# SyamVangara/multigrid-petsc

Hardware: AMD Instinct MI355X
Metric: fp64 DOF-updates/sec per V-cycle at 1024^3 (higher is better)
Workload: dtype f64

## Files before the change

### include/mgk.h

```cpp
#ifndef MGK_H
#define MGK_H
#include <stddef.h>
#ifdef __cplusplus
extern "C" {
#endif

#define MGK_XOFF 16
#define MGK_EINVAL  10001
#define MGK_ENOGPU  10002
#define MGK_ECOMM   10003

typedef struct mgk_ctx mgk_ctx;

typedef struct mgk_geom {
    int  dim;
    int  nx, ny, nz;
    int  pitch;
    long plane;
    long org;
    long total;
} mgk_geom;

int  mgk_geom_init(mgk_geom *g, int dim, int nx, int ny, int nz);

// ... 348 lines not shown
    MGK_TUNE_J2_REG_PRED       = 36,
    MGK_TUNE_J2_RING_PRED      = 37,
    MGK_TUNE_PJ2D_WAVES        = 38,
    MGK_TUNE_J2_RING_OLD       = 39,
    MGK_TUNE_SRR_TY2           = 40,
    MGK_TUNE_SRR_TY4           = 41,
    MGK_TUNE_J2_ZERO_RINGB     = 45,
    MGK_TUNE_PJ2_COPY          = 46,
    MGK_TUNE_J3_2D_MARCH       = 50,
    MGK_TUNE_J3_2D_CHUNK4      = 51,
    MGK_TUNE_J3_2D_CHUNK8      = 52,
    MGK_TUNE_DISPATCH_ORDER    = 53,
    MGK_TUNE_XCD_ORDER         = 54,
    MGK_TUNE_RR2D_MARCH        = 55,
    MGK_TUNE_RR2D_SHORT        = 56,
    MGK_TUNE_RESERVED_57       = 57,
    MGK_TUNE_J3_2D_ODD_DOWN    = 58,
    MGK_TUNE_J3_2D_ALL_DOWN    = 59,
    MGK_TUNE_J3_2D_STORE_PLAIN = 60,
    MGK_TUNE_J3_2D_STORE_NT    = 61,
    MGK_TUNE_J3_3D_TY2         = 62,
    MGK_TUNE_J3_3D_TY3         = 63,
    MGK_TUNE_J3_3D_ROWWISE     = 64,
    MGK_TUNE_NO_EXACT_FMA      = 65
};

void mgk_set_tuning(int variant, int zchunk);

#ifdef __cplusplus
}
#endif
#endif
```

### multigrid_petsc_amd/csrc/mg_solver.c

```c
#include "mgsolve.h"
#include "mg_comm.h"
#include "mg_solver_internal.h"
#include <math.h>
#include <stdio.h>
#include <stdlib.h>
#include <string.h>
#include <time.h>

#define MG_PI 3.14159265358979323846
static __thread char g_mgerr[512] = "ok";
const char *mg_last_error(void) { return g_mgerr; }
static int mgfail(int code, const char *what) {
    snprintf(g_mgerr, sizeof(g_mgerr), "%s (code %d; kernel layer: %s)", what, code, mgk_last_error());
    return code;
}

typedef struct mg_ops {
    int esz;
    int (*jacobi_range)(mgk_ctx *, const mgk_geom *, const double *, double, double, const void *, const void *, void *, int, int, void *);
    int (*jacobi_zero)(mgk_ctx *, const mgk_geom *, double, double, const void *, void *, void *);
    int (*residual)(mgk_ctx *, const mgk_geom *, const double *, const void *, const void *, void *, void *);
    int (*restrict_fw)(mgk_ctx *, const mgk_geom *, const mgk_geom *, const void *, void *, void *);
    int (*prolong_add)(mgk_ctx *, const mgk_geom *, const mgk_geom *, const void *, void *, void *);
    int (*prolong_jacobi)(mgk_ctx *, const mgk_geom *, const mgk_geom *, const double *, double, double, const void *, const void *, const void *, void *, void *);
// ... 295 lines not shown
    if (s->cfg.rtol <= 0) s->cfg.rtol = 1.e-7;
    if (s->cfg.dist_min_n <= 0) {
        const int n0 = mg_grid_n(cfg->npts, 0);
        s->cfg.dist_min_n = n0 < 255 ? n0 : 255;
    }
    if (s->cfg.fuse < 0) s->cfg.fuse = MG_FUSE_DEFAULT;
    if (s->cfg.pair_min_n <= 0) s->cfg.pair_min_n = (cfg->dim == 3) ? 255 : 2047;
    if (s->cfg.pc_type == MG_PC_RBGS) s->cfg.fuse &= ~(MG_FUSE_POINT_JACOBI_PASSES & ~MG_FUSE_PROLONG_SWEEP);
    else if (s->cfg.pc_type != MG_PC_JACOBI) s->cfg.fuse &= ~MG_FUSE_POINT_JACOBI_PASSES;
    if (s->cfg.mesh) s->cfg.fuse &= ~MG_FUSE_NO_ROW_TABLE_FORM;
    if (s->cfg.overlap < 0) s->cfg.overlap = 1;
    if (s->cfg.graph < 0) s->cfg.graph = 1;
    if (s->cfg.nranks < 1) s->cfg.nranks = 1;
    s->comm = comm;
    s->levels = cfg->levels;
    int rc = mgk_ctx_create(&s->ctx, cfg->device);
    if (rc) { free(s); return mgfail(rc, "mg_solver_create: mgk_ctx_create"); }
    if (s->cfg.slab_chunk < 0) {
        const char *e = getenv("MG_SLAB_CHUNK");
        const int quarter = (mg_grid_n(cfg->npts, 0) / (s->cfg.nranks > 0 ? s->cfg.nranks : 1)) / 4;
        s->cfg.slab_chunk = (e && *e && atoi(e) >= 0) ? atoi(e) : (quarter > 32 ? quarter : 32);
    }
    if (s->cfg.nranks > 1 && s->cfg.dim == 3) mgk_ctx_set_chunk_planes(s->ctx, s->cfg.slab_chunk);

    s->ldist = 0;
    if (s->cfg.nranks > 1) {
        for (int l = 0; l < s->levels; l++) {
            int n = mg_grid_n(cfg->npts, l);
            if (n >= s->cfg.dist_min_n && n >= 2 * s->cfg.nranks) s->ldist = l + 1; else break;
        }
        if (s->ldist == 0) { mg_solver_destroy(s); return mgfail(MGK_EINVAL, "mg_solver_create: grid too small to distribute"); }
        s->zstart = (int *)calloc(s->cfg.nranks + 1, sizeof(int));
        for (int r = 0; r < s->cfg.nranks; r++) {
            int a, b;
            if (mg_slab_range(cfg->npts, s->ldist, s->ldist, r, s->cfg.nranks, &a, &b)) {
                mg_solver_destroy(s);
                return mgfail(MGK_EINVAL, "mg_solver_create: too many ranks for this grid");
            }
            s->zstart[r] = a; s->zstart[r + 1] = b;
        }
    }

    const int mixed = (cfg->precision == MG_PREC_MIXED);
    for (int l = 0; l < s->levels; l++) {
        mg_level *L = &s->L[l];
        L->n = mg_grid_n(cfg->npts, l);
// ... 576 lines not shown
    }
    CHK(O->restrict_fw(s->ctx, &F->g, &Cq->g, F->rv, Cq->b, NULL));
    return 0;
}

static int prolong_from(mg_solver *s, int P, int l) {
    mg_level *Lf = &s->L[l], *Lc = &s->L[l + 1];
    mg_fset *F = &Lf->f[P], *Cq = &Lc->f[P];
    const mg_ops *O = &OPS[P];
    if (F->u_ghost_pending) CHK(ensure_u_ghosts(s, P, Lf));
    if (Lf->distributed && !Lc->distributed) {
        mgk_geom gc = Cq->g;
        int c0 = s->zstart[s->cfg.rank], c1 = s->zstart[s->cfg.rank + 1];
        gc.nz = c1 - c0;
        CHK(O->prolong_add(s->ctx, &F->g, &gc, (char *)Cq->u + (size_t)O->esz * (size_t)c0 * (size_t)Cq->g.plane, F->u, NULL));
    } else {
        CHK(ensure_u_ghosts(s, P, Lc));
        CHK(O->prolong_add(s->ctx, &F->g, &Cq->g, Cq->u, F->u, NULL));
    }
    F->u_ghost_ok = 0;
    return 0;
}

static int pjp_ok(const mg_solver *s, int P) {
    const mg_level *L = &s->L[0];
    const int need = MG_FUSE_PROLONG_PAIR | MG_FUSE_SWEEP_RESTRICT | MG_FUSE_PAIRS | MG_FUSE_NORM_SWEEP | MG_FUSE_PROLONG_SWEEP | MG_FUSE_RESNORM;
    if ((s->cfg.fuse & need) != need || P != 0 || s->cfg.dim != 3 || s->cfg.mesh || s->cfg.ksp_type != MG_KSP_RICHARDSON) return 0;
    if (s->cfg.v[0] != 3 || s->levels < 2 || s->lgraph == 1 || L->n < s->cfg.pair_min_n || s->last_cycle) return 0;
    if (L->distributed) {
        const mg_level *Lc = &s->L[1];
        const int hi = s->cfg.rank < s->cfg.nranks - 1;
        if (!(s->cfg.fuse & MG_FUSE_PROLONG_PAIR_SLAB) || !Lc->distributed || !L->f[0].far || !Lc->f[0].far || L->nz_min < 8 || Lc->nz_min < 4) return 0;
        return mgk_prolong_jacobi2_slab_ok_f64(&L->f[0].g, &Lc->f[0].g, hi) && mgk_jacobi2_sumsq_ok_f64(&L->f[0].g);
    }
    return mgk_prolong_jacobi2_ok_f64(&L->f[0].g, &s->L[1].f[0].g) && mgk_jacobi2_sumsq_ok_f64(&L->f[0].g);
}
static int finalize_iterate(mg_solver *s) {
    if (!s->iterate_behind) return 0;
    mg_level *L = &s->L[0];
    mg_fset *F = &L->f[0];
    if (L->distributed) {
        CHK(ensure_u_ghosts(s, 0, L));
        CHK(mgk_jacobi_range_f64(s->ctx, &F->g, L->coef, L->dinv, s->cfg.scale, (const double *)F->b, (const double *)F->u, (double *)F->tmp, 0, F->g.nz, NULL));
    } else
    CHK(mgk_jacobi_f64(s->ctx, &F->g, L->coef, L->dinv, s->cfg.scale, (const double *)F->b, (const double *)F->u, (double *)F->tmp, NULL));
    swap_ptr(&F->u, &F->tmp);
    mgi_u_rewritten(F);
    s->iterate_behind = 0; s->spec_valid = 0;
    return 0;
}

// ... 342 lines not shown
        if (s->sweep_owed && L->distributed) {
            const int nz = F->g.nz, lo = s->cfg.rank > 0, hi = s->cfg.rank < s->cfg.nranks - 1;
            void *cs = mgk_stream_compute(s->ctx), *ms = mgk_stream_comm(s->ctx);
            int n1 = 0, n2 = 0, n3 = 0;
            CHK(group_exchange(s, 0, F, 0));
#define J2M(z0, z1, off, np) mgk_jacobi2_sumsq_mid_slab_f64(s->ctx, &F->g, &F->gfar, L->coef, L->dinv, s->cfg.scale, (const double *)F->b, (const double *)F->u, \
                                (double *)F->tmp, (const double *)F->far, lo, hi, z0, z1, off, np, cs)
            const int split = s->cfg.overlap && nz >= 6;
            if (split) {
                void *t = prof_begin_kind(s, 0, 1);
                int rc2 = J2M(2, nz - 2, 0, &n1);
                prof_end(s, t);
                CHK(rc2);
            }
            CHK(mgk_stream_wait(s->ctx, cs, ms));
            F->u_ghost_pending = 0; F->u_ghost_ok = 1; F->b_ghost_ok = 1;
            if (split) { CHK(J2M(0, 2, n1, &n2)); CHK(J2M(nz - 2, nz, n1 + n2, &n3)); }
            else CHK(J2M(0, nz, 0, &n1));
#undef J2M
            CHK(mgk_partials_finish(s->ctx, n1 + n2 + n3, &ss, NULL));
            s->sweep_owed = 0; s->iterate_behind = 1; s->spec_valid = 1;
            goto norm_done;
        }
        if (s->sweep_owed) {
            void *t = prof_begin_kind(s, 0, 1);
            int rc2 = mgk_jacobi2_sumsq_mid_f64(s->ctx, &F->g, L->coef, L->dinv, s->cfg.scale, (const double *)F->b, (const double *)F->u,
                                                (double *)F->tmp, &ss, NULL);
            prof_end(s, t);
            CHK(rc2);
            s->sweep_owed = 0; s->iterate_behind = 1; s->spec_valid = 1;
            goto norm_done;
        }
        if (jnorm && L->distributed && s->cfg.dim == 3 && (s->cfg.fuse & MG_FUSE_SWEEP_RESTRICT) && (s->cfg.fuse & MG_FUSE_PAIRS) && F->far && L->nz_min >= 6 &&
            s->cfg.v[0] >= 2 && L->n >= s->cfg.pair_min_n && L->n + 1 <= 1024 && s->lgraph != 1 && mgk_jacobi2_sumsq_ok_f64(&F->g)) {
            const int nz = F->g.nz, lo = s->cfg.rank > 0, hi = s->cfg.rank < s->cfg.nranks - 1;
            void *cs = mgk_stream_compute(s->ctx), *ms = mgk_stream_comm(s->ctx);
            int n1 = 0, n2 = 0, n3 = 0;
            CHK(group_exchange(s, 0, F, 0));
#define J2N(z0, z1, off, np) mgk_jacobi2_sumsq_slab_f64(s->ctx, &F->g, &F->gfar, L->coef, L->dinv, s->cfg.scale, (const double *)F->b, (const double *)F->u, \
                                (double *)F->tmp, (const double *)F->far, lo, hi, z0, z1, off, np, cs)
            const int split = s->cfg.overlap && nz >= 6;
            if (split) CHK(J2N(2, nz - 2, 0, &n1));
            CHK(mgk_stream_wait(s->ctx, cs, ms));
            F->u_ghost_pending = 0; F->u_ghost_ok = 1; F->b_ghost_ok = 1;
            if (split) { CHK(J2N(0, 2, n1, &n2)); CHK(J2N(nz - 2, nz, n1 + n2, &n3)); }
            else CHK(J2N(0, nz, 0, &n1));
// ... 80 lines not shown
    else CHK(mgk_residual_sumsq_f64(s->ctx, &F->g, L->coef, (const double *)F->b, (const double *)F->u, &ss, NULL));
    CHK(norm_from_sumsq(s, ss, &s->rchk));
    s->spec_valid = 0; s->sweep_owed = 0; s->iterate_behind = 0;
    s->iter = 0;
    s->rnorm[0] = s->rchk;
    s->started = 1;
    return 0;
}

int mg_solver_reset(mg_solver *s) { s->started = 0; s->iter = 0; return 0; }

static double wall(void) {
    struct timespec t;
    clock_gettime(CLOCK_MONOTONIC, &t);
    return t.tv_sec + 1e-9 * t.tv_nsec;
}

int mgi_iterate(mg_solver *s) {
    const int devnorm = s->cfg.nranks > 1 && s->comm->allreduce_sum_dev != NULL;
    if (devnorm) CHK(need_slots(s, 1));
    while (s->iter < s->cfg.maxiter && 100000000 * s->bnorm > s->rchk && s->rchk > s->cfg.rtol * s->bnorm) {
        s->last_cycle = (s->iter + 1 >= s->cfg.maxiter) ||
                        (s->iter >= 1 && s->rnorm[s->iter - 1] > 0.0 && s->rchk * (s->rchk / s->rnorm[s->iter - 1]) <= s->cfg.rtol * s->bnorm);
        if (!devnorm) { int rc1 = vcycle_once(s); s->last_cycle = 0; CHK(rc1); continue; }
        double ss = 0.0;
        int rc = mgk_defer_result(s->ctx, s->d_norms);
        s->deferring = 1;
        if (!rc) rc = vcycle_once(s);
        s->deferring = 0;
        s->last_cycle = 0;
        mgk_defer_result(s->ctx, NULL);
        if (rc) return rc;
        CHK(reduce_slots(s, s->d_norms, 1, &ss));
        s->rchk = sqrt(ss);
        if (s->iter < s->rnorm_cap) s->rnorm[s->iter] = s->rchk;
    }
    return 0;
}

int mg_solver_solve(mg_solver *s) {
    CHK(start(s));
    CHK(mgk_sync(s->ctx, NULL));
    double t0 = wall();
    CHK(mgi_iterate(s));
    CHK(finalize_iterate(s));
    CHK(mgk_sync(s->ctx, NULL));
    s->solve_seconds = wall() - t0;
    return 0;
}

int mg_solver_cycles(mg_solver *s, int ncycles) {
    if (!s->started) CHK(start(s));
    if (s->iter + ncycles >= s->rnorm_cap) {
        int cap = s->iter + ncycles + 1;
        double *r = (double *)realloc(s->rnorm, sizeof(double) * (size_t)cap);
        if (!r) return mgfail(MGK_EINVAL, "mg_solver_cycles: out of host memory");
        s->rnorm = r; s->rnorm_cap = cap;
    }
    CHK(need_slots(s, ncycles));
    const int it0 = s->iter;
    s->deferring = 1;
    int rc = 0;
    for (int q = 0; q < ncycles && !rc; q++) {
        rc = mgk_defer_result(s->ctx, s->d_norms + q);
        s->last_cycle = (q == ncycles - 1);
        if (!rc) rc = vcycle_once(s);
    }
    s->last_cycle = 0;
    mgk_defer_result(s->ctx, NULL);
    s->deferring = 0;
    if (!rc) rc = finalize_iterate(s);
    if (rc) return rc;
    double *ss = (double *)malloc(sizeof(double) * (size_t)(ncycles > 0 ? ncycles : 1));
    if (!ss) return mgfail(MGK_EINVAL, "mg_solver_cycles: out of host memory");
    rc = reduce_slots(s, s->d_norms, ncycles, ss);
    if (rc) { free(ss); return mgfail(rc, "mg_solver_cycles: reading the deferred norms"); }
    for (int q = 0; q < ncycles; q++) s->rnorm[it0 + 1 + q] = sqrt(ss[q]);
    if (ncycles > 0) s->rchk = s->rnorm[it0 + ncycles];
    free(ss);
    return 0;
}

int mg_solver_sync(mg_solver *s) {
    CHK(mgk_sync(s->ctx, NULL));
    if (s->comm && s->comm->check) { int rcc = s->comm->check(s->comm); if (rcc) return mgfail(rcc, mg_comm_last_error()); }
    return 0;
}
int mg_solver_iterations(const mg_solver *s) { return s->iter; }
double mg_solver_bnorm(const mg_solver *s) { return s->bnorm; }
const double *mg_solver_rnorm(const mg_solver *s) { return s->rnorm; }
double mg_solver_solve_seconds(const mg_solver *s) { return s->solve_seconds; }
// ... 55 lines not shown
```

### multigrid_petsc_amd/csrc/mg_solver_internal.h

```cpp
#ifndef MG_SOLVER_INTERNAL_H
#define MG_SOLVER_INTERNAL_H
#include "mgsolve.h"
#include "mg_comm.h"
#include "mg_cheby_coefs.h"

#define MG_MAX_LEVELS 32
#define MG_MAX_TIMERS 4096

#define MG_FUSE_POINT_JACOBI_PASSES (MG_FUSE_PROLONG_SWEEP | MG_FUSE_NORM_SWEEP | MG_FUSE_PAIRS | MG_FUSE_COARSE_ZERO_SWEEP | MG_FUSE_LDS_TAIL | \
                                     MG_FUSE_SWEEP_RESTRICT | MG_FUSE_ZERO_TRIPLE | MG_FUSE_PROLONG_PAIR | MG_FUSE_TRIPLE_2D | \
                                     MG_FUSE_PROLONG_PAIR_SLAB | MG_FUSE_CHEBY)
#define MG_FUSE_NO_ROW_TABLE_FORM   (MG_FUSE_MIXED_CORRECT | MG_FUSE_RES_RESTRICT_SMALL)

typedef struct mg_fset {
    mgk_geom g;
    void *u, *b, *rv, *tmp;
    int guess_nonzero;
    int u_ghost_ok;
    int u_ghost_pending;
    int jz_ready;
    int last_sweep_pending;
    int b_ghost_ok;
    int pre_done;
    void *far;
// ... 18 lines not shown
    double *chunktab;
    double *xchunktab, *xchunksep;
} mg_level;

struct mg_solver {
    mg_config cfg;
    mgk_ctx *ctx;
    mg_comm *comm;
    int levels, ldist;
    mg_level L[MG_MAX_LEVELS];
    int *zstart;
    double *rnorm;
    int rnorm_cap;
    int iter;
    double bnorm, rchk;
    int started;
    int deferring;
    double *d_norms; int d_norms_cap;
    double *pin; int pin_cap;
    int spec_valid;
    int sweep_owed;
    int last_cycle;
    int iterate_behind;
    double solve_seconds;
    int lgraph;
    int ltail;
    void *coarse_graph[2];
    void *graph_u[2], *graph_tmp[2];
    int graph_rerecorded;
    int prof_on, prof_n;
    void *timers[MG_MAX_TIMERS];
    unsigned char timer_kind[MG_MAX_TIMERS];
    int prof_kind;
    int ntimers_created;
    void *gm_field[MGK_KRYLOV_MAX + 3];
    int gm_nfields, gm_restart;
    double *gm_hdev;
};

enum { MG_CHEBY_ZERO = 0, MG_CHEBY_PLAIN = 1, MG_CHEBY_PROLONG = 2, MG_CHEBY_NORM = 3 };
extern int mg_cheby_pass(mg_solver *s, int l, int kind, double *sumsq) __attribute__((weak));
extern int mg_cheby_tail(mg_solver *s) __attribute__((weak));

extern int mg_line_tables(mg_solver *s, int l, const double *ctab_host) __attribute__((weak));
extern int mg_line_smooth(mg_solver *s, int l, int maxit) __attribute__((weak));
extern int mg_xline_tables(mg_solver *s, int l, const double *ctab_host) __attribute__((weak));
extern int mg_xline_smooth(mg_solver *s, int l, int maxit) __attribute__((weak));
extern int mg_line_chunk_tables(mg_solver *s, int l, const double *ctab_host) __attribute__((weak));
extern int mg_line_chunk_smooth(mg_solver *s, int l, int maxit) __attribute__((weak));
extern int mg_xline_chunk_tables(mg_solver *s, int l, const double *ctab_host) __attribute__((weak));
extern int mg_xline_chunk_smooth(mg_solver *s, int l, int maxit) __attribute__((weak));
extern int mg_line_tail(mg_solver *s) __attribute__((weak));
extern int mg_rbgs_smooth(mg_solver *s, int l, int maxit) __attribute__((weak));
extern int mg_rbgs_prolong_smooth(mg_solver *s, int l, int maxit) __attribute__((weak));
long mg_xline_stride(int n, int uniform);
void mg_xline_factor(int n, int rows, const double *ctab, long gs, double *g);

int    mgi_fail(int code, const char *what);
#define CHK(call) do { int rc_ = (call); if (rc_) return mgi_fail(rc_, #call); } while (0)
int    mgi_upload(mg_solver *s, const double *h, size_t n, double **d);
double mgi_wall(void);
int    mgi_start(mg_solver *s);
int    mgi_smooth(mg_solver *s, int l, int maxit);
int    mgi_vcycle_rooted(mg_solver *s, int l);
int    mgi_vcycle_once(mg_solver *s);
int    mgi_iterate(mg_solver *s);
int    mgi_finalize(mg_solver *s);
int    mgi_apply_cycle(mg_solver *s);
#endif
```

### multigrid_petsc_amd/csrc/mgk_kernels.hip

```cpp
#include "mgk_dev.hpp"

thread_local char g_err[512] = "ok";
int fail(int code, const char *what) {
    snprintf(g_err, sizeof(g_err), "%s (code %d%s%s)", what, code,
             code < 10000 ? ": " : "", code < 10000 ? hipGetErrorString((hipError_t)code) : "");
    return code;
}
const void *g_preload_kernels[MGK_PRELOAD_MAX];
int g_preload_count;


extern "C" const char *mgk_last_error(void) { return g_err; }

extern "C" int mgk_device_count(void) {
    int n = 0;
    if (hipGetDeviceCount(&n) != hipSuccess) return 0;
    return n;
}

extern "C" int mgk_set_device(int device) { HIPCHK(hipSetDevice(device)); return 0; }

static void ctx_release(mgk_ctx *c) {
    if (c->partials) (void)hipFree(c->partials);
    if (c->result_dev) (void)hipFree(c->result_dev);
// ... 1279 lines not shown
                    const T Wv = ring[sc][q][xl + VX - 1], Ev = ring[sc][q][xl + 2 * VX];
                    VT o = jac7(a.a0, a.a1, a.a2, a.a3, a.a4, a.a5, a.a6, a.dinv, a.scale, dn, sv, c, nv, upv, Wv, Ev, b0[j]);
                    if (lastlane) o.v[VX - 1] = (T)0;
                    bufst_nt<T>(o, ro, lb, (unsigned)(yb + j + 1) * rowb);
                }
            }
        }
        __syncthreads();
#pragma unroll
        for (int j = 0; j < TY; j++) b0[j] = b1[j + 1];
#pragma unroll
        for (int q = 0; q < R2; q++) b1[q] = bn[q];
#pragma unroll
        for (int rr = 0; rr < R1; rr++) D[rr] = first(D[rr]);
    };
    for (int t = t0; t < z1; t += 4) {
        step(ua, ub, uc, ud, t);
        if (t + 1 < z1) step(ub, uc, ud, ua, t + 1);
        if (t + 2 < z1) step(uc, ud, ua, ub, t + 2);
        if (t + 3 < z1) step(ud, ua, ub, uc, t + 3);
    }
}

template <typename T, int WX, int FORM, int NORM = 0, bool EX = false>
__global__ void __launch_bounds__(64 * WX) k_jacobi2r(const J2Args<T> a) {
    constexpr bool UNC = (FORM & 1) != 0, DPP = (FORM & 2) != 0;
    constexpr int VX = 16 / sizeof(T), TY = 4, R1 = TY + 4, R2 = TY + 2, TX = 64 * VX * WX, LW = TX + 2 * VX;
    __shared__ __attribute__((aligned(16))) T cen[2][R2][LW];
    __shared__ T edgeW[2][R2][WX], edgeE[2][R2][WX];
    using VT = V16<T>;
    const int tid = threadIdx.x, lane = tid & 63, w = tid >> 6;
    int bid = blockIdx.x;
    const int nblk = gridDim.x;
    if ((nblk & 7) == 0) bid = (bid & 7) * (nblk >> 3) + (bid >> 3);
    const int ty = bid % a.nty, tz = bid / a.nty;
    const int yb = TY * ty;
    const int z0 = a.zbeg + tz * a.zc, z1 = min(z0 + a.zc, a.zend);
    if (z0 >= z1) { if (NORM && tid == 0) a.partials[blockIdx.x] = 0.0; return; }
    const int xl = VX * tid, x0 = xl;
    const bool xok = x0 < a.nx;
    const bool lastvec = (x0 + VX > a.nx);

    bool uok[R1], s1ok[R2];
#pragma unroll
    for (int rr = 0; rr < R1; rr++) { const int y = yb - 2 + rr; uok[rr] = xok && y >= -1 && y <= a.ny; }
#pragma unroll
    for (int q = 0; q < R2; q++) { const int y = yb - 1 + q; s1ok[q] = y >= 0 && y < a.ny; }
// ... 10 lines not shown
#pragma unroll
    for (int rr = 0; rr < R1; rr++) uro[rr] = (long)max(-1, min(yb - 2 + rr, a.ny)) * a.rs;
#pragma unroll
    for (int q = 0; q < R2; q++) bro[q] = (long)max(0, min(yb - 1 + q, a.ny)) * a.rs;
    auto LDU = [&](int p, int rr, bool pv) -> VT {
        if (UNC) {
            const int pp = max(pmin, min(p, pmax));
            const T *pl = (pp == -2) ? a.far_lo : (pp == a.nz + 1) ? a.far_hi : a.u + (long)pp * a.ms;
            return *reinterpret_cast<const VT *>(reinterpret_cast<const char *>(pl + uro[rr]) + lb);
        }
        return ldv(uplane(p) + (long)rr * a.rs, uok[rr] && pv);
    };
    auto LDB = [&](int p, int q, bool pv, bool stream) -> VT {
        if (UNC) {
            const T *pl = a.b + (long)max(smin, min(p, smax)) * a.ms + bro[q];
            const T *ad = reinterpret_cast<const T *>(reinterpret_cast<const char *>(pl) + lb);
            return stream ? ldv_stream(ad, true) : ldv(ad, true);
        }
        const T *bp = bp_ + (long)p * a.ms + (long)q * a.rs;
        const bool ok = xok && s1ok[q] && pv;
        return stream ? ldv_stream(bp, ok) : ldv(bp, ok);
    };

    VT ua[R1], ub[R1], uc[R1], b1[R2], bn[R2], b0[TY], wm[TY], wc[TY], wp[TY];
    double nacc = 0.0;
    const int t0 = z0 - 2;
#pragma unroll
    for (int rr = 0; rr < R1; rr++) {
        const long ro = (long)rr * a.rs;
        (void)ro;
        ua[rr] = LDU(t0, rr, t0 >= pmin);
        ub[rr] = LDU(t0 + 1, rr, t0 + 1 >= pmin);
        uc[rr] = LDU(t0 + 2, rr, true);
    }
#pragma unroll
    for (int q = 0; q < R2; q++) {
        const int p = t0 + 1;
        b1[q] = LDB(p, q, p >= smin && p <= smax, false);
        bn[q] = v16_zero<T>();
    }
#pragma unroll
    for (int j = 0; j < TY; j++) { b0[j] = v16_zero<T>(); wm[j] = b0[j]; wc[j] = b0[j]; wp[j] = b0[j]; }
    if (lane == 0 || lane == 63) {
#pragma unroll
        for (int q = 0; q < R2; q++) {
            if (lane == 0) edgeW[(t0 + 1) & 1][q][w] = ub[q + 1].v[0];
            else edgeE[(t0 + 1) & 1][q][w] = ub[q + 1].v[VX - 1];
        }
    }
    __syncthreads();

    for (int t = t0; t < z1; t++) {
        const int p = t + 1;
        {
            const bool pb = (t + 2 <= smax) && (t + 1 < z1);
#pragma unroll
// ... 11 lines not shown
                VT o;
#pragma unroll
                for (int e = 0; e < VX; e++) {
                    const T wv = (e == 0) ? Wv : ub[rr].v[e - 1 < 0 ? 0 : e - 1];
                    const T ev = (e == VX - 1) ? Ev : ub[rr].v[e + 1 > VX - 1 ? VX - 1 : e + 1];
                    T s = a.a0 * ua[rr].v[e];
                    s = madd<EX>(s, a.a1, ub[rr - 1].v[e]);
                    s = madd<EX>(s, a.a2, wv);
                    s = s + a.a3 * ub[rr].v[e];
                    s = madd<EX>(s, a.a4, ev);
                    s = madd<EX>(s, a.a5, ub[rr + 1].v[e]);
                    s = madd<EX>(s, a.a6, uc[rr].v[e]);
                    const T res = b1[q].v[e] - s;
                    const T zz = res * a.dinv;
                    o.v[e] = ub[rr].v[e] + a.scale * zz;
                    if (!pin || !s1ok[q] || !xok || (lastvec && x0 + e >= a.nx)) o.v[e] = (T)0;
                    if (NORM == 1 && q >= 1 && q <= TY) {
                        const bool own = (p >= z0 && p < z1) && s1ok[q] && xok && !(lastvec && x0 + e >= a.nx);
                        nacc += own ? (double)res * (double)res : 0.0;
                    }
                }
                *reinterpret_cast<VT *>(&cen[cb][q][xl + VX]) = o;
                if (q >= 1 && q <= TY) wp[q - 1] = o;
            }
            if (lane == 0 || lane == 63) {
#pragma unroll
                for (int q = 0; q < R2; q++) {
                    if (lane == 0) edgeW[eb ^ 1][q][w] = uc[q + 1].v[0];
                    else edgeE[eb ^ 1][q][w] = uc[q + 1].v[VX - 1];
                }
            }
        }
        {
            const bool pu = (t + 3 <= pmax);
#pragma unroll
            for (int rr = 0; rr < R1; rr++) ua[rr] = LDU(t + 3, rr, pu);
        }
        if (t >= z0) {
            const int cb = t & 1;
#pragma unroll
            for (int j = 0; j < TY; j++) {
                const int q = j + 1;
                const VT sv = *reinterpret_cast<const VT *>(&cen[cb][q - 1][xl + VX]);
                const VT nv = *reinterpret_cast<const VT *>(&cen[cb][q + 1][xl + VX]);
                const T Wv = cen[cb][q][xl + VX - 1], Ev = cen[cb][q][xl + 2 * VX];
                VT o;
#pragma unroll
                for (int e = 0; e < VX; e++) {
                    const T wv = (e == 0) ? Wv : wc[j].v[e - 1 < 0 ? 0 : e - 1];
                    const T ev = (e == VX - 1) ? Ev : wc[j].v[e + 1 > VX - 1 ? VX - 1 : e + 1];
                    T s = a.a0 * wm[j].v[e];
                    s = madd<EX>(s, a.a1, sv.v[e]);
                    s = madd<EX>(s, a.a2, wv);
                    s = s + a.a3 * wc[j].v[e];
                    s = madd<EX>(s, a.a4, ev);
                    s = madd<EX>(s, a.a5, nv.v[e]);
                    s = madd<EX>(s, a.a6, wp[j].v[e]);
                    const T res = b0[j].v[e] - s;
                    const T zz = res * a.dinv;
                    o.v[e] = wc[j].v[e] + a.scale * zz;
                    if (lastvec && x0 + e >= a.nx) o.v[e] = (T)0;
                    if (NORM == 2) nacc += (xok && yb + j < a.ny && !(lastvec && x0 + e >= a.nx)) ? (double)res * (double)res : 0.0;
                }
                if (xok && yb + j < a.ny) stv_stream(a.out + (long)t * a.ms + (long)(yb + j) * a.rs + x0, o);
            }
        }
        __syncthreads();
#pragma unroll
        for (int j = 0; j < TY; j++) { b0[j] = b1[j + 1]; wm[j] = wc[j]; wc[j] = wp[j]; }
#pragma unroll
        for (int q = 0; q < R2; q++) b1[q] = bn[q];
#pragma unroll
        for (int rr = 0; rr < R1; rr++) { VT tmpv = ua[rr]; ua[rr] = ub[rr]; ub[rr] = uc[rr]; uc[rr] = tmpv; }
    }
    if (NORM) {
        double *red = reinterpret_cast<double *>(&cen[0][0][0]);
        __syncthreads();
        const double sblk = block_sum(nacc, red);
        if (tid == 0) a.partials[blockIdx.x] = sblk;
    }
}



struct PJ2Args {
    const double *u, *b, *uc;
    double *out;
    int nx, ny, nz, nxc, nyc, nzc;
    long rs, ms, crs, cms;
    int nty, zc;
    double a0, a1, a2, a3, a4, a5, a6, dinv, scale;
    const double *far_lo, *far_hi, *cfar_lo;
    int has_lo, has_hi, zbeg, zend;
};
typedef unsigned int mgk_u2v __attribute__((ext_vector_type(2)));
template <int WX>
// ... 494 lines not shown
    J2Args<T> a; memset(&a, 0, sizeof(a));
    a.u = u + g->org; a.b = b + g->org; a.out = unew + g->org;
    a.nx = g->nx; a.ny = g->ny; a.nz = g->nz; a.rs = g->pitch; a.ms = g->plane;
    set_coef7(a, coef);
    a.dinv = (T)dinv; a.scale = (T)scale;
    a.far_lo = far_lo; a.far_hi = far_hi; a.has_lo = far_lo != nullptr; a.has_hi = far_hi != nullptr;
    if (zbeg < 0 || zend > g->nz || zbeg >= zend) return fail(MGK_EINVAL, "mgk_jacobi2: empty or out-of-range plane range");
    a.zbeg = zbeg; a.zend = zend;
    const int nzr = zend - zbeg;
    a.nty = (g->ny + 3) / 4;
    const int w = (g->nx + 1 + 64 * VX - 1) / (64 * VX);
    const long target = (w > 4) ? 256 : ((sizeof(T) == 4 || w <= 2) ? 1024 : 512);
    const Chunks ch = cut_chunks(c, nzr, a.nty, target, { 8, false,  false,  true,  1, 1});
    a.zc = ch.len;
    const unsigned nblk = (unsigned)(a.nty * ch.count);
    hipStream_t s = S(c, stream);
    if (norm_parts) {
        constexpr int WRn = 64 * VX;
        if (sizeof(T) != 8 || (g->nx + 1) % WRn != 0 || (g->ny + 1) % 4 != 0 || part_off < 0 || (long)nblk > c->max_partials - part_off)
            return fail(MGK_EINVAL, "mgk_jacobi2_sumsq: built for fp64 full-row shapes (n = 127, 255, 511, 1023)");
        a.partials = c->partials + part_off;
        if constexpr (sizeof(T) == 8) {
            const bool exn = exact_fma7(coef);
            if (norm_mode == 2) LAUNCH_WX_EX(width_1248, w, T, exn, (k_jacobi2r<T, WX, 3, 2, EX>), nblk, s, a);
            else LAUNCH_WX_EX(width_1248, w, T, exn, (k_jacobi2r<T, WX, 3, 1, EX>), nblk, s, a);
        }
        HIPCHK(hipGetLastError());
        *norm_parts = (int)nblk;
        return 0;
    }
    const bool ring = (g_variant == 1) || (g_variant == MGK_TUNE_J2_RING_PRED) || (g_variant != 2 && g_variant != MGK_TUNE_J2_REG_PRED && !(sizeof(T) == 8 && w > 4));
    constexpr int WR = 64 * VX;
    const bool full = (g->nx + 1) % WR == 0 && (g->ny + 1) % 4 == 0 && g_variant != MGK_TUNE_J2_REG_PRED && g_variant != MGK_TUNE_J2_RING_PRED;
    if (zero_guess) {
        if (!full || far_lo || far_hi || norm_parts) return fail(MGK_EINVAL, "mgk_jacobi2_zero: built for whole grids of full-row shape (the LDS-ring form of the two-sweep kernel)");
        if (g_variant == MGK_TUNE_J2_RING_OLD || (sizeof(T) == 8 && g_variant != MGK_TUNE_J2_ZERO_RINGB)) {
            LAUNCH_WX(width_1248, w, (k_jacobi2<T, WX, 3, true>), nblk, s, a);
        } else LAUNCH_WX(width_1248, w, (k_jacobi2b<T, WX, true>), nblk, s, a);
        HIPCHK(hipGetLastError());
        return 0;
    }
    if (ring) {
        if (full && g_variant != MGK_TUNE_J2_RING_OLD) {
            LAUNCH_WX(width_1248, w, (k_jacobi2b<T, WX, false>), nblk, s, a);
        } else if (full) {
            LAUNCH_WX(width_1248, w, (k_jacobi2<T, WX, 3>), nblk, s, a);
        } else {
            LAUNCH_WX(width_1248, w, (k_jacobi2<T, WX, 0>), nblk, s, a);
        }
    } else {
        if (full) {
            LAUNCH_WX_EX(width_1248, w, T, exact_fma7(coef), (k_jacobi2r<T, WX, 3, 0, EX>), nblk, s, a);
        } else {
            LAUNCH_WX(width_1248, w, (k_jacobi2r<T, WX, 0>), nblk, s, a);
        }
    }
    HIPCHK(hipGetLastError());
    return 0;
// ... 24 lines not shown
    return jacobi2<double>(c, g, coef, dinv, scale, b, nullptr, unew, nullptr, nullptr, 0, g->nz, stream, nullptr, 0, true);
}
extern "C" int mgk_jacobi2_zero_f32(mgk_ctx *c, const mgk_geom *g, const double *coef, double dinv, double scale,
                                    const float *b, float *unew, void *stream) {
    if (!g) return fail(MGK_EINVAL, "mgk_jacobi2_zero_f32: bad arguments");
    return jacobi2<float>(c, g, coef, dinv, scale, b, nullptr, unew, nullptr, nullptr, 0, g->nz, stream, nullptr, 0, true);
}
extern "C" int mgk_jacobi2_sumsq_ok_f64(const mgk_geom *g) {
    return (g && g->dim == 3 && (g->nx + 1) % 128 == 0 && (g->ny + 1) % 4 == 0 && g->nx + 1 <= 1024) ? 1 : 0;
}
extern "C" int mgk_jacobi2_sumsq_f64(mgk_ctx *c, const mgk_geom *g, const double *coef, double dinv, double scale,
                                     const double *b, const double *u, double *unew, double *sumsq_host, void *stream) {
    if (!g || !sumsq_host) return fail(MGK_EINVAL, "mgk_jacobi2_sumsq_f64: bad arguments");
    int nparts = 0;
    int rc = jacobi2<double>(c, g, coef, dinv, scale, b, u, unew, nullptr, nullptr, 0, g->nz, stream, &nparts);
    if (rc) return rc;
    return finish_to_host(c, nparts, 1, S(c, stream), sumsq_host);
}
extern "C" int mgk_jacobi2_sumsq_mid_f64(mgk_ctx *c, const mgk_geom *g, const double *coef, double dinv, double scale,
                                         const double *b, const double *u, double *unew, double *sumsq_host, void *stream) {
    if (!g || !sumsq_host) return fail(MGK_EINVAL, "mgk_jacobi2_sumsq_mid_f64: bad arguments");
    int nparts = 0;
    int rc = jacobi2<double>(c, g, coef, dinv, scale, b, u, unew, nullptr, nullptr, 0, g->nz, stream, &nparts, 0, false, 2);
    if (rc) return rc;
    return finish_to_host(c, nparts, 1, S(c, stream), sumsq_host);
}
extern "C" int mgk_jacobi2_sumsq_slab_f64(mgk_ctx *c, const mgk_geom *g, const mgk_geom *gfar, const double *coef, double dinv, double scale,
                                          const double *b, const double *u, double *unew, const double *far, int has_lo, int has_hi,
                                          int zbeg, int zend, int part_off, int *nparts, void *stream) {
    if (!g || !nparts) return fail(MGK_EINVAL, "mgk_jacobi2_sumsq_slab_f64: bad arguments");
    if ((has_lo || has_hi) && !(far_geom_ok(gfar, far, g) && g->nz >= 2))
        return fail(MGK_EINVAL, "mgk_jacobi2_sumsq_slab_f64: the far-plane field must have the geometry (nx, ny, 2) of the slab");
    const double *lo = far_lo_plane(far, gfar, has_lo), *hi = far_hi_plane(far, gfar, has_hi);
    return jacobi2<double>(c, g, coef, dinv, scale, b, u, unew, lo, hi, zbeg, zend, stream, nparts, part_off);
}
extern "C" int mgk_jacobi2_sumsq_mid_slab_f64(mgk_ctx *c, const mgk_geom *g, const mgk_geom *gfar, const double *coef, double dinv, double scale,
                                              const double *b, const double *u, double *unew, const double *far, int has_lo, int has_hi,
                                              int zbeg, int zend, int part_off, int *nparts, void *stream) {
    if (!g || !nparts) return fail(MGK_EINVAL, "mgk_jacobi2_sumsq_mid_slab_f64: bad arguments");
    if ((has_lo || has_hi) && !(far_geom_ok(gfar, far, g) && g->nz >= 2))
        return fail(MGK_EINVAL, "mgk_jacobi2_sumsq_mid_slab_f64: the far-plane field must have the geometry (nx, ny, 2) of the slab");
    const double *lo = far_lo_plane(far, gfar, has_lo), *hi = far_hi_plane(far, gfar, has_hi);
    return jacobi2<double>(c, g, coef, dinv, scale, b, u, unew, lo, hi, zbeg, zend, stream, nparts, part_off, false, 2);
}
template <typename T>
static int jacobi2_slab(mgk_ctx *c, const mgk_geom *g, const mgk_geom *gfar, const double *coef, double dinv, double scale,
// ... 2652 lines not shown
```

### multigrid_petsc_amd/mgk.py

```python
import contextlib
import ctypes as C
import enum
import numpy as np
from ._lib import load_mgk

c_dp = C.POINTER(C.c_double)


class Geom(C.Structure):
    _fields_ = [("dim", C.c_int), ("nx", C.c_int), ("ny", C.c_int), ("nz", C.c_int),
                ("pitch", C.c_int), ("plane", C.c_long), ("org", C.c_long), ("total", C.c_long)]


class MgkError(RuntimeError):
    pass


class Tune(enum.IntEnum):
    DEFAULT = -1
    STORE_PLAIN = 0
    STORE_NT = 1
    LDS_TILE = 30
    ROW = 31
    ROW_PD2 = 32
# ... 4 lines not shown
    J2_RING_PRED = 37
    PJ2D_WAVES = 38
    J2_RING_OLD = 39
    SRR_TY2 = 40
    SRR_TY4 = 41
    J2_ZERO_RINGB = 45
    PJ2_COPY = 46
    J3_2D_MARCH = 50
    J3_2D_CHUNK4 = 51
    J3_2D_CHUNK8 = 52
    DISPATCH_ORDER = 53
    XCD_ORDER = 54
    RR2D_MARCH = 55
    RR2D_SHORT = 56
    RESERVED_57 = 57
    J3_2D_ODD_DOWN = 58
    J3_2D_ALL_DOWN = 59
    J3_2D_STORE_PLAIN = 60
    J3_2D_STORE_NT = 61
    J3_3D_TY2 = 62
    J3_3D_TY3 = 63
    J3_3D_ROWWISE = 64
    NO_EXACT_FMA = 65


@contextlib.contextmanager
def tuning(variant=-1, zchunk=-1):
    L = load_mgk()
    L.mgk_set_tuning.restype, L.mgk_set_tuning.argtypes = None, [C.c_int, C.c_int]
    L.mgk_set_tuning(int(variant), int(zchunk))
    try:
        yield
    finally:
        L.mgk_set_tuning(-1, -1)


def _sigs(L):
    vp, i, d, sz = C.c_void_p, C.c_int, C.c_double, C.c_size_t
    G = C.POINTER(Geom)
    S = {
        "mgk_geom_init": (i, [G, i, i, i, i]),
        "mgk_device_count": (i, []),
        "mgk_set_device": (i, [i]),
        "mgk_ctx_create": (i, [C.POINTER(vp), i]),
        "mgk_ctx_destroy": (None, [vp]),
        "mgk_last_error": (C.c_char_p, []),
# ... 72 lines not shown
        "mgk_flat_axpbypcz": (i, [vp, C.c_long, d, d, d, vp, vp, vp, vp]),
        "mgk_flat_pointwise_mult": (i, [vp, C.c_long, vp, vp, vp, vp]),
        "mgk_defer_result": (i, [vp, vp]),
        "mgk_csr_mult_f64": (i, [vp, C.c_long, vp, vp, vp, vp, vp, d, vp, i, C.c_long, C.c_long, vp]),
        "mgk_jacobi_zero_rowcoef_f64": (i, [vp, G, vp, d, vp, vp, vp]),
        "mgk_rowcoef_f64": (i, [vp, G, i, vp, vp, d, vp, vp, vp, vp]),
        "mgk_cheby_rowcoef_f64": (i, [vp, G, vp, vp, d, d, d, vp, vp, vp, vp, vp]),
        "mgk_jacobi_range_f64": (i, [vp, G, c_dp, d, d, vp, vp, vp, i, i, vp]),
        "mgk_jacobi2_slab_f64": (i, [vp, G, G, c_dp, d, d, vp, vp, vp, vp, i, i, i, i, vp]),
        "mgk_prolong_jacobi_f64": (i, [vp, G, G, c_dp, d, d, vp, vp, vp, vp, vp]),
        "mgk_prolong_jacobi_f32": (i, [vp, G, G, c_dp, d, d, vp, vp, vp, vp, vp]),
        "mgk_prolong_jacobi_range_f64": (i, [vp, G, G, c_dp, d, d, vp, vp, vp, vp, i, i, vp]),
        "mgk_prolong_jacobi_range_f32": (i, [vp, G, G, c_dp, d, d, vp, vp, vp, vp, i, i, vp]),
        "mgk_residual_restrict_range_f64": (i, [vp, G, G, c_dp, vp, vp, vp, i, i, vp]),
        "mgk_residual_restrict_range_f32": (i, [vp, G, G, c_dp, vp, vp, vp, i, i, vp]),
        "mgk_residual_restrict_slab_f64": (i, [vp, G, G, G, c_dp, vp, vp, vp, i, vp, i, i, vp]),
        "mgk_residual_restrict_slab_f32": (i, [vp, G, G, G, c_dp, vp, vp, vp, i, vp, i, i, vp]),
        "mgk_residual_restrict_2d_f64": (i, [vp, G, G, c_dp, vp, vp, vp, vp, d, d, vp]),
        "mgk_sweep_residual_restrict_f64": (i, [vp, G, G, c_dp, d, d, vp, vp, vp, vp, vp, d, d, vp]),
        "mgk_sweep_residual_restrict_ok_f64": (i, [G, G]),
        "mgk_jacobi2_sumsq_f64": (i, [vp, G, c_dp, d, d, vp, vp, vp, C.POINTER(d), vp]),
        "mgk_jacobi2_sumsq_ok_f64": (i, [G]),
        "mgk_jacobi2_sumsq_mid_f64": (i, [vp, G, c_dp, d, d, vp, vp, vp, C.POINTER(d), vp]),
        "mgk_prolong_jacobi2_ok_f64": (i, [G, G]),
        "mgk_prolong_jacobi2_f64": (i, [vp, G, G, c_dp, d, d, vp, vp, vp, vp, vp]),
        "mgk_jacobi2_zero_ok_f64": (i, [G]),
        "mgk_jacobi2_zero_ok_f32": (i, [G]),
        "mgk_jacobi2_zero_f64": (i, [vp, G, c_dp, d, d, vp, vp, vp]),
        "mgk_jacobi2_zero_f32": (i, [vp, G, c_dp, d, d, vp, vp, vp]),
        "mgk_jacobi2_2d_sumsq_f64": (i, [vp, G, c_dp, d, d, vp, vp, vp, C.POINTER(d), vp]),
        "mgk_jacobi3_f64": (i, [vp, G, c_dp, d, d, vp, vp, vp, vp]),
        "mgk_jacobi3_sumsq_f64": (i, [vp, G, c_dp, d, d, vp, vp, vp, C.POINTER(d), vp]),
        "mgk_jacobi3_2d_f64": (i, [vp, G, c_dp, d, d, vp, vp, vp, vp, vp, vp]),
        "mgk_jacobi3_2d_sumsq_f64": (i, [vp, G, c_dp, d, d, vp, vp, vp, vp, vp, C.POINTER(d), vp]),
        "mgk_jacobi3_2d_zero_f64": (i, [vp, G, c_dp, d, d, vp, vp, vp, vp, vp]),
        "mgk_jacobi3_2d_sumsq_store_f64": (i, [vp, G, c_dp, d, d, vp, vp, vp, vp, vp, vp, C.POINTER(d), vp]),
        "mgk_prolong_jacobi3_2d_f64": (i, [vp, G, G, c_dp, d, d, vp, vp, vp, vp, vp, vp, vp]),
        "mgk_cheby3_2d_f64": (i, [vp, G, c_dp, d, c_dp, vp, vp, vp, vp, vp, vp]),
        "mgk_cheby3_2d_sumsq_f64": (i, [vp, G, c_dp, d, c_dp, vp, vp, vp, vp, vp, C.POINTER(d), vp]),
        "mgk_cheby3_2d_zero_f64": (i, [vp, G, c_dp, d, c_dp, vp, vp, vp, vp, vp]),
        "mgk_prolong_cheby3_2d_f64": (i, [vp, G, G, c_dp, d, c_dp, vp, vp, vp, vp, vp, vp, vp]),
        "mgk_tail_cycle_cheby_f64": (i, [vp, G, i, C.POINTER(i), c_dp, c_dp, C.POINTER(vp), C.POINTER(vp), d, d, i, i, vp, vp, vp]),
        "mgk_sweep_residual_restrict_2d_f64": (i, [vp, G, G, c_dp, d, d, vp, vp, vp, vp, vp, d, d, vp]),
        "mgk_jacobi2_sumsq_slab_f64": (i, [vp, G, G, c_dp, d, d, vp, vp, vp, vp, i, i, i, i, i, C.POINTER(i), vp]),
        "mgk_jacobi2_sumsq_mid_slab_f64": (i, [vp, G, G, c_dp, d, d, vp, vp, vp, vp, i, i, i, i, i, C.POINTER(i), vp]),
        "mgk_prolong_jacobi2_slab_ok_f64": (i, [G, G, i]),
# ... 159 lines not shown
```

Baseline: 382.6 billion.

## Add last-cycle close pass and register-ring zero-guess two-sweep Jacobi

On the final V-cycle the fused prolong/Jacobi pair path is now allowed, and the owed sweep is finished by a new NORM==3 variant of the two-sweep kernel. That variant stores only the first sweep and computes the residual norm of the second without writing it, so the deferred iterate and the extra finalize sweep are no longer needed. Separately, the zero-initial-guess two-sweep path for fp64 with width 4 or 8 now uses the register-ring k_jacobi2r kernel, with the first sweep folded into the loads. The two features can be disabled by an environment variable and a tuning variant respectively. Both add code paths whose numerics and boundary handling must match the old kernels.

Result: no change. 383.7 billion (median of 6 runs) (+0.3%).

```diff
diff --git a/include/mgk.h b/include/mgk.h
--- a/include/mgk.h
+++ b/include/mgk.h
@@ -394,7 +394,8 @@
     MGK_TUNE_J3_3D_TY2         = 62,
     MGK_TUNE_J3_3D_TY3         = 63,
     MGK_TUNE_J3_3D_ROWWISE     = 64,
-    MGK_TUNE_NO_EXACT_FMA      = 65
+    MGK_TUNE_NO_EXACT_FMA      = 65,
+    MGK_TUNE_J2_ZERO_RING      = 66
 };
 
 void mgk_set_tuning(int variant, int zchunk);
diff --git a/multigrid_petsc_amd/csrc/mg_close.c b/multigrid_petsc_amd/csrc/mg_close.c
--- /dev/null
+++ b/multigrid_petsc_amd/csrc/mg_close.c
@@ -0,0 +1,13 @@
+#include "mg_solver_internal.h"
+#include "mgk_close.h"
+#include <stddef.h>
+
+int mg_close_pass(mg_solver *s, double *sumsq) {
+    mg_level *L = &s->L[0];
+    mg_fset *F = &L->f[0];
+    if (!sumsq) return mgi_fail(MGK_EINVAL, "mg_close_pass: the pass needs a destination for the norm");
+    if (L->distributed || s->cfg.dim != 3 || !F->tmp) return mgi_fail(MGK_EINVAL, "mg_close_pass: built for whole 3-D grids in fp64");
+    CHK(mgk_jacobi2_sumsq_close_f64(s->ctx, &F->g, L->coef, L->dinv, s->cfg.scale, (const double *)F->b, (const double *)F->u, (double *)F->tmp,
+                                    sumsq, NULL));
+    return 0;
+}
diff --git a/multigrid_petsc_amd/csrc/mg_solver.c b/multigrid_petsc_amd/csrc/mg_solver.c
--- a/multigrid_petsc_amd/csrc/mg_solver.c
+++ b/multigrid_petsc_amd/csrc/mg_solver.c
@@ -341,6 +341,10 @@
         s->cfg.slab_chunk = (e && *e && atoi(e) >= 0) ? atoi(e) : (quarter > 32 ? quarter : 32);
     }
     if (s->cfg.nranks > 1 && s->cfg.dim == 3) mgk_ctx_set_chunk_planes(s->ctx, s->cfg.slab_chunk);
+    {
+        const char *e = getenv("MG_CLOSE_PASS");
+        s->close_on = !(e && *e && atoi(e) == 0);
+    }
 
     s->ldist = 0;
     if (s->cfg.nranks > 1) {
@@ -963,11 +967,14 @@
     return 0;
 }
 
+static int close_ok(const mg_solver *s) {
+    return s->close_armed && s->close_on && mg_close_pass && !s->L[0].distributed;
+}
 static int pjp_ok(const mg_solver *s, int P) {
     const mg_level *L = &s->L[0];
     const int need = MG_FUSE_PROLONG_PAIR | MG_FUSE_SWEEP_RESTRICT | MG_FUSE_PAIRS | MG_FUSE_NORM_SWEEP | MG_FUSE_PROLONG_SWEEP | MG_FUSE_RESNORM;
     if ((s->cfg.fuse & need) != need || P != 0 || s->cfg.dim != 3 || s->cfg.mesh || s->cfg.ksp_type != MG_KSP_RICHARDSON) return 0;
-    if (s->cfg.v[0] != 3 || s->levels < 2 || s->lgraph == 1 || L->n < s->cfg.pair_min_n || s->last_cycle) return 0;
+    if (s->cfg.v[0] != 3 || s->levels < 2 || s->lgraph == 1 || L->n < s->cfg.pair_min_n || (s->last_cycle && !close_ok(s))) return 0;
     if (L->distributed) {
         const mg_level *Lc = &s->L[1];
         const int hi = s->cfg.rank < s->cfg.nranks - 1;
@@ -1356,6 +1363,16 @@
             s->sweep_owed = 0; s->iterate_behind = 1; s->spec_valid = 1;
             goto norm_done;
         }
+        if (s->sweep_owed && s->last_cycle) {
+            void *t = prof_begin_kind(s, 0, 1);
+            int rc2 = mg_close_pass(s, &ss);
+            prof_end(s, t);
+            CHK(rc2);
+            swap_ptr(&F->u, &F->tmp);
+            mgi_u_rewritten(F);
+            s->sweep_owed = 0; s->iterate_behind = 0; s->spec_valid = 0;
+            goto norm_done;
+        }
         if (s->sweep_owed) {
             void *t = prof_begin_kind(s, 0, 1);
             int rc2 = mgk_jacobi2_sumsq_mid_f64(s->ctx, &F->g, L->coef, L->dinv, s->cfg.scale, (const double *)F->b, (const double *)F->u,
@@ -1482,13 +1499,14 @@
     while (s->iter < s->cfg.maxiter && 100000000 * s->bnorm > s->rchk && s->rchk > s->cfg.rtol * s->bnorm) {
         s->last_cycle = (s->iter + 1 >= s->cfg.maxiter) ||
                         (s->iter >= 1 && s->rnorm[s->iter - 1] > 0.0 && s->rchk * (s->rchk / s->rnorm[s->iter - 1]) <= s->cfg.rtol * s->bnorm);
-        if (!devnorm) { int rc1 = vcycle_once(s); s->last_cycle = 0; CHK(rc1); continue; }
+        s->close_armed = s->last_cycle;
+        if (!devnorm) { int rc1 = vcycle_once(s); s->last_cycle = 0; s->close_armed = 0; CHK(rc1); continue; }
         double ss = 0.0;
         int rc = mgk_defer_result(s->ctx, s->d_norms);
         s->deferring = 1;
         if (!rc) rc = vcycle_once(s);
         s->deferring = 0;
-        s->last_cycle = 0;
+        s->last_cycle = 0; s->close_armed = 0;
         mgk_defer_result(s->ctx, NULL);
         if (rc) return rc;
         CHK(reduce_slots(s, s->d_norms, 1, &ss));
@@ -1524,9 +1542,10 @@
     for (int q = 0; q < ncycles && !rc; q++) {
         rc = mgk_defer_result(s->ctx, s->d_norms + q);
         s->last_cycle = (q == ncycles - 1);
+        s->close_armed = s->last_cycle;
         if (!rc) rc = vcycle_once(s);
     }
-    s->last_cycle = 0;
+    s->last_cycle = 0; s->close_armed = 0;
     mgk_defer_result(s->ctx, NULL);
     s->deferring = 0;
     if (!rc) rc = finalize_iterate(s);
diff --git a/multigrid_petsc_amd/csrc/mg_solver_internal.h b/multigrid_petsc_amd/csrc/mg_solver_internal.h
--- a/multigrid_petsc_amd/csrc/mg_solver_internal.h
+++ b/multigrid_petsc_amd/csrc/mg_solver_internal.h
@@ -64,6 +64,8 @@
     int sweep_owed;
     int last_cycle;
     int iterate_behind;
+    int close_armed;
+    int close_on;
     double solve_seconds;
     int lgraph;
     int ltail;
@@ -95,6 +97,7 @@
 extern int mg_line_tail(mg_solver *s) __attribute__((weak));
 extern int mg_rbgs_smooth(mg_solver *s, int l, int maxit) __attribute__((weak));
 extern int mg_rbgs_prolong_smooth(mg_solver *s, int l, int maxit) __attribute__((weak));
+extern int mg_close_pass(mg_solver *s, double *sumsq) __attribute__((weak));
 long mg_xline_stride(int n, int uniform);
 void mg_xline_factor(int n, int rows, const double *ctab, long gs, double *g);
 
diff --git a/multigrid_petsc_amd/csrc/mgk_close.h b/multigrid_petsc_amd/csrc/mgk_close.h
--- /dev/null
+++ b/multigrid_petsc_amd/csrc/mgk_close.h
@@ -0,0 +1,12 @@
+#ifndef MGK_CLOSE_H
+#define MGK_CLOSE_H
+#include "mgk.h"
+#ifdef __cplusplus
+extern "C" {
+#endif
+int  mgk_jacobi2_sumsq_close_f64(mgk_ctx *ctx, const mgk_geom *g, const double *coef, double dinv, double scale,
+                                 const double *b, const double *u, double *unew, double *sumsq_host, void *stream);
+#ifdef __cplusplus
+}
+#endif
+#endif
diff --git a/multigrid_petsc_amd/csrc/mgk_kernels.hip b/multigrid_petsc_amd/csrc/mgk_kernels.hip
--- a/multigrid_petsc_amd/csrc/mgk_kernels.hip
+++ b/multigrid_petsc_amd/csrc/mgk_kernels.hip
@@ -1,4 +1,5 @@
 #include "mgk_dev.hpp"
+#include "mgk_close.h"
 
 thread_local char g_err[512] = "ok";
 int fail(int code, const char *what) {
@@ -1325,7 +1326,7 @@
     }
 }
 
-template <typename T, int WX, int FORM, int NORM = 0, bool EX = false>
+template <typename T, int WX, int FORM, int NORM = 0, bool EX = false, bool ZG = false>
 __global__ void __launch_bounds__(64 * WX) k_jacobi2r(const J2Args<T> a) {
     constexpr bool UNC = (FORM & 1) != 0, DPP = (FORM & 2) != 0;
     constexpr int VX = 16 / sizeof(T), TY = 4, R1 = TY + 4, R2 = TY + 2, TX = 64 * VX * WX, LW = TX + 2 * VX;
@@ -1382,6 +1383,14 @@
         return stream ? ldv_stream(bp, ok) : ldv(bp, ok);
     };
 
+    auto first = [&](VT v) -> VT {
+        if (ZG) {
+#pragma unroll
+            for (int e = 0; e < VX; e++) { const T zx = v.v[e] * a.dinv; v.v[e] = a.scale * zx; }
+        }
+        return v;
+    };
+
     VT ua[R1], ub[R1], uc[R1], b1[R2], bn[R2], b0[TY], wm[TY], wc[TY], wp[TY];
     double nacc = 0.0;
     const int t0 = z0 - 2;
@@ -1389,9 +1398,9 @@
     for (int rr = 0; rr < R1; rr++) {
         const long ro = (long)rr * a.rs;
         (void)ro;
-        ua[rr] = LDU(t0, rr, t0 >= pmin);
-        ub[rr] = LDU(t0 + 1, rr, t0 + 1 >= pmin);
-        uc[rr] = LDU(t0 + 2, rr, true);
+        ua[rr] = first(LDU(t0, rr, t0 >= pmin));
+        ub[rr] = first(LDU(t0 + 1, rr, t0 + 1 >= pmin));
+        uc[rr] = first(LDU(t0 + 2, rr, true));
     }
 #pragma unroll
     for (int q = 0; q < R2; q++) {
@@ -1449,6 +1458,9 @@
                 }
                 *reinterpret_cast<VT *>(&cen[cb][q][xl + VX]) = o;
                 if (q >= 1 && q <= TY) wp[q - 1] = o;
+                if (NORM == 3 && q >= 1 && q <= TY) {
+                    if (p >= z0 && p < z1 && xok && yb + q - 1 < a.ny) stv_stream(a.out + (long)p * a.ms + (long)(yb + q - 1) * a.rs + x0, o);
+                }
             }
             if (lane == 0 || lane == 63) {
 #pragma unroll
@@ -1484,12 +1496,14 @@
                     s = madd<EX>(s, a.a5, nv.v[e]);
                     s = madd<EX>(s, a.a6, wp[j].v[e]);
                     const T res = b0[j].v[e] - s;
-                    const T zz = res * a.dinv;
-                    o.v[e] = wc[j].v[e] + a.scale * zz;
-                    if (lastvec && x0 + e >= a.nx) o.v[e] = (T)0;
-                    if (NORM == 2) nacc += (xok && yb + j < a.ny && !(lastvec && x0 + e >= a.nx)) ? (double)res * (double)res : 0.0;
+                    if (NORM != 3) {
+                        const T zz = res * a.dinv;
+                        o.v[e] = wc[j].v[e] + a.scale * zz;
+                        if (lastvec && x0 + e >= a.nx) o.v[e] = (T)0;
+                    }
+                    if (NORM >= 2) nacc += (xok && yb + j < a.ny && !(lastvec && x0 + e >= a.nx)) ? (double)res * (double)res : 0.0;
                 }
-                if (xok && yb + j < a.ny) stv_stream(a.out + (long)t * a.ms + (long)(yb + j) * a.rs + x0, o);
+                if (NORM != 3 && xok && yb + j < a.ny) stv_stream(a.out + (long)t * a.ms + (long)(yb + j) * a.rs + x0, o);
             }
         }
         __syncthreads();
@@ -1498,7 +1512,7 @@
 #pragma unroll
         for (int q = 0; q < R2; q++) b1[q] = bn[q];
 #pragma unroll
-        for (int rr = 0; rr < R1; rr++) { VT tmpv = ua[rr]; ua[rr] = ub[rr]; ub[rr] = uc[rr]; uc[rr] = tmpv; }
+        for (int rr = 0; rr < R1; rr++) { VT tmpv = ua[rr]; ua[rr] = ub[rr]; ub[rr] = uc[rr]; uc[rr] = first(tmpv); }
     }
     if (NORM) {
         double *red = reinterpret_cast<double *>(&cen[0][0][0]);
@@ -2039,7 +2053,8 @@
         a.partials = c->partials + part_off;
         if constexpr (sizeof(T) == 8) {
             const bool exn = exact_fma7(coef);
-            if (norm_mode == 2) LAUNCH_WX_EX(width_1248, w, T, exn, (k_jacobi2r<T, WX, 3, 2, EX>), nblk, s, a);
+            if (norm_mode == 3) LAUNCH_WX_EX(width_1248, w, T, exn, (k_jacobi2r<T, WX, 3, 3, EX>), nblk, s, a);
+            else if (norm_mode == 2) LAUNCH_WX_EX(width_1248, w, T, exn, (k_jacobi2r<T, WX, 3, 2, EX>), nblk, s, a);
             else LAUNCH_WX_EX(width_1248, w, T, exn, (k_jacobi2r<T, WX, 3, 1, EX>), nblk, s, a);
         }
         HIPCHK(hipGetLastError());
@@ -2051,6 +2066,13 @@
     const bool full = (g->nx + 1) % WR == 0 && (g->ny + 1) % 4 == 0 && g_variant != MGK_TUNE_J2_REG_PRED && g_variant != MGK_TUNE_J2_RING_PRED;
     if (zero_guess) {
         if (!full || far_lo || far_hi || norm_parts) return fail(MGK_EINVAL, "mgk_jacobi2_zero: built for whole grids of full-row shape (the LDS-ring form of the two-sweep kernel)");
+        if constexpr (sizeof(T) == 8) {
+            if ((w == 8 || w == 4) && g_variant != MGK_TUNE_J2_ZERO_RING && g_variant != MGK_TUNE_J2_RING_OLD && g_variant != MGK_TUNE_J2_ZERO_RINGB) {
+                LAUNCH_WX_EX(width_48, w, T, exact_fma7(coef), (k_jacobi2r<T, WX, 3, 0, EX, true>), nblk, s, a);
+                HIPCHK(hipGetLastError());
+                return 0;
+            }
+        }
         if (g_variant == MGK_TUNE_J2_RING_OLD || (sizeof(T) == 8 && g_variant != MGK_TUNE_J2_ZERO_RINGB)) {
             LAUNCH_WX(width_1248, w, (k_jacobi2<T, WX, 3, true>), nblk, s, a);
         } else LAUNCH_WX(width_1248, w, (k_jacobi2b<T, WX, true>), nblk, s, a);
@@ -2121,6 +2143,14 @@
     if (!g || !sumsq_host) return fail(MGK_EINVAL, "mgk_jacobi2_sumsq_mid_f64: bad arguments");
     int nparts = 0;
     int rc = jacobi2<double>(c, g, coef, dinv, scale, b, u, unew, nullptr, nullptr, 0, g->nz, stream, &nparts, 0, false, 2);
+    if (rc) return rc;
+    return finish_to_host(c, nparts, 1, S(c, stream), sumsq_host);
+}
+extern "C" int mgk_jacobi2_sumsq_close_f64(mgk_ctx *c, const mgk_geom *g, const double *coef, double dinv, double scale,
+                                           const double *b, const double *u, double *unew, double *sumsq_host, void *stream) {
+    if (!g || !sumsq_host) return fail(MGK_EINVAL, "mgk_jacobi2_sumsq_close_f64: bad arguments");
+    int nparts = 0;
+    int rc = jacobi2<double>(c, g, coef, dinv, scale, b, u, unew, nullptr, nullptr, 0, g->nz, stream, &nparts, 0, false, 3);
     if (rc) return rc;
     return finish_to_host(c, nparts, 1, S(c, stream), sumsq_host);
 }
diff --git a/multigrid_petsc_amd/mgk.py b/multigrid_petsc_amd/mgk.py
--- a/multigrid_petsc_amd/mgk.py
+++ b/multigrid_petsc_amd/mgk.py
@@ -50,6 +50,7 @@
     J3_3D_TY3 = 63
     J3_3D_ROWWISE = 64
     NO_EXACT_FMA = 65
+    J2_ZERO_RING = 66
 
 
 @contextlib.contextmanager
@@ -168,6 +169,7 @@
         "mgk_jacobi2_sumsq_f64": (i, [vp, G, c_dp, d, d, vp, vp, vp, C.POINTER(d), vp]),
         "mgk_jacobi2_sumsq_ok_f64": (i, [G]),
         "mgk_jacobi2_sumsq_mid_f64": (i, [vp, G, c_dp, d, d, vp, vp, vp, C.POINTER(d), vp]),
+        "mgk_jacobi2_sumsq_close_f64": (i, [vp, G, c_dp, d, d, vp, vp, vp, C.POINTER(d), vp]),
         "mgk_prolong_jacobi2_ok_f64": (i, [G, G]),
         "mgk_prolong_jacobi2_f64": (i, [vp, G, G, c_dp, d, d, vp, vp, vp, vp, vp]),
         "mgk_jacobi2_zero_ok_f64": (i, [G]),
```
